# k-flouris/cmf

Measured on AMD Instinct MI355X. Metric: log-density evals/sec (JtJ-cholesky path), MNIST D=784 d=64 bs=512, higher is better.
Workload: dtype f32 (3x3 tangent convs as bf16x3 split MFMA, fp32 accumulate); 1 GPU; C3: MNIST-shaped (1,28,28) uint8-range + U[0,1) noise, non-square flow d=64, cholesky J^T J log-det + g_ij off-diagonal L1 + reconstruction, eval/no_grad; per_gpu_batch=512, global_batch=512, D=784, latent_dimension=64, parallelism=dp1

## Files before the change

### cmf_amd/_lib.py

```python
import ctypes as C
import os
import threading

_HERE = os.path.dirname(os.path.abspath(__file__))
LIB_PATH = os.path.join(_HERE, "libcmf_amd.so")

F_NONE, F_RELU, F_TANH, F_RAW, F_SELF_RELU, F_RELU_BITS = 0, 1, 2, 3, 4, 5
O_NONE, O_TANH, O_STANH = 0, 1, 2

_fp = C.c_void_p
_ll = C.c_longlong
_i = C.c_int
_f = C.c_float
_d = C.c_double


class ConvTangentArgs(C.Structure):
    _fields_ = [("x", _fp), ("x_np", _ll), ("x_ci", _ll), ("x_px", _ll),
                ("f", _fp), ("f_np", _ll), ("f_ci", _ll), ("f_px", _ll), ("fmode", _i),
                ("w", _fp),
                ("y", _fp), ("y_np", _ll), ("y_co", _ll), ("y_px", _ll),
                ("r", _fp), ("r_np", _ll), ("r_co", _ll), ("r_px", _ll),
                ("np", _i), ("cin", _i), ("cout", _i), ("H", _i), ("W", _i), ("nc", _i), ("taps", _i),
                ("bias", _fp), ("f_group", _i), ("x_sl", _ll), ("y_sl", _ll), ("r_sl", _ll),
                ("fo", _fp), ("fo_np", _ll), ("fo_co", _ll), ("fo_px", _ll), ("fomode", _i),
                ("mask_out", _fp), ("mask_np", _ll), ("amax_in", _fp), ("amax_out", _fp), ("live", _i),
                ("ymask", _fp), ("ymask_np", _ll),
                ("head_w", _fp), ("head_cout", _i), ("head_a", _fp), ("head_a_np", _ll), ("head_a_c", _ll), ("head_a_px", _ll),
                ("head_y", _fp), ("head_y_np", _ll), ("head_y_co", _ll), ("head_y_px", _ll)]


class ConvPrimalArgs(C.Structure):
    _fields_ = [("x", _fp), ("x_b", _ll), ("x_c", _ll), ("x_px", _ll),
                ("f", _fp), ("f_c", _ll), ("f_px", _ll), ("imode", _i),
                ("w", _fp), ("bias", _fp), ("sw", _fp), ("sb", _fp),
                ("y", _fp), ("y_b", _ll), ("y_c", _ll), ("y_px", _ll),
                ("g", _fp),
                ("r", _fp), ("r_b", _ll), ("r_c", _ll), ("r_px", _ll),
                ("omode", _i),
                ("B", _i), ("cin", _i), ("cout", _i), ("H", _i), ("W", _i), ("taps", _i)]


class ProbeApplyArgs(C.Structure):
    _fields_ = [("r", _fp), ("r_np", _ll), ("r_px", _ll),
# ... 12 lines not shown
    _fields_ = [("z", _fp), ("z_b", _ll), ("t", _fp), ("t_f", _ll), ("w", _fp),
                ("zi", _fp), ("si", _fp), ("ti", _fp), ("n_mod", _i),
                ("B", _i), ("cin", _i), ("chan_off", _i), ("chan_step", _i), ("n_layers", _i),
                ("width", _i * (MLP_MAX_LAYERS + 1)), ("w_off", _ll * MLP_MAX_LAYERS), ("decode", _i), ("lj", _fp), ("ncols", _i)]


SIGNATURES = {
    "cmf_version": (C.c_char_p, []),
    "cmf_pack_weight": (_i, [_fp, _fp, _i, _i, _i, _i, C.POINTER(_ll), _fp]),
    "cmf_pack_weights_batched": (_i, [_fp, _i, _fp]),
    "cmf_conv_tangent": (_i, [C.POINTER(ConvTangentArgs), _fp]),
    "cmf_pack_weight_bf16x3": (_i, [_fp, _fp, _i, _i, C.POINTER(_ll), _fp]),
    "cmf_pack_weight_bf16x3_t": (_i, [_fp, _fp, _i, _i, _i, C.POINTER(_ll), _fp]),
    "cmf_conv_tangent_bf16x3": (_i, [C.POINTER(ConvTangentArgs), _fp]),
    "cmf_probe_apply": (_i, [C.POINTER(ProbeApplyArgs), _fp]),
    "cmf_pack_weight_f16x3": (_i, [_fp, _fp, _i, _i, _i, C.POINTER(_ll), _fp]),
    "cmf_conv_tangent_f16x3": (_i, [C.POINTER(ConvTangentArgs), _fp]),
    "cmf_conv_tangent_f16x3_item": (_i, [C.POINTER(ConvTangentArgs), _i, _fp]),
    "cmf_absmax": (_i, [_fp, _ll, _fp, _fp]),
    "cmf_conv_tangent_wgrad_ws": (_ll, [C.POINTER(ConvTangentArgs)]),
    "cmf_conv_tangent_wgrad": (_i, [C.POINTER(ConvTangentArgs), _fp, _fp, _fp, _ll, _fp]),
    "cmf_conv_tangent_wgrad_bf16x3": (_i, [C.POINTER(ConvTangentArgs), _fp, _fp, _fp, _ll, _fp]),
    "cmf_conv_tangent_wgrad_bf16x3_batched": (_i, [C.POINTER(ConvTangentArgs), _i, C.POINTER(_fp), C.POINTER(_fp), C.POINTER(_fp), _fp, _ll, _fp]),
    "cmf_primal_regroup": (_i, [_fp, _fp, _i, _ll, _i, _fp]),
    "cmf_conv_primal": (_i, [C.POINTER(ConvPrimalArgs), _fp]),
    "cmf_acl_primal": (_i, [_fp, _ll, _fp, _ll, _fp, _fp, _fp, _i, _i, _i, _fp, _fp]),
    "cmf_acl_tangent": (_i, [_fp, _ll, _ll, _fp, _ll, _ll, _i, _fp, _ll, _fp, _ll, _fp, _fp, _fp, _fp, _i, _i, _fp]),
    "cmf_acl_cotangent": (_i, [_fp, _ll, _ll, _fp, _ll, _ll, _i, _fp, _ll, _fp, _ll, _fp, _fp, _fp, _fp, _i, _i, _fp]),
    "cmf_acl_primal_backward": (_i, [_fp, _ll, _fp, _ll, _fp, _ll, _fp, _fp, _fp, _fp, _i, _i, _i, _fp, _fp]),
    "cmf_acl_cross_terms": (_i, [_fp, _ll, _ll, _fp, _ll, _ll, _fp, _ll, _ll, _i, _fp, _ll, _fp, _ll, _fp, _fp, _fp, _fp, _i, _i,
# ... 138 lines not shown
```

### cmf_amd/csrc/conv_tangent_bf16x3.hip

```cpp
#include <cstdlib>
#include <type_traits>
#include "common.h"

#ifdef CMF_DBG_STAMP
__device__ unsigned long long cmf_dbg_stamps[3][64][4];
extern "C" int cmf_debug_read_stamps(void* out) {
  return (int)hipMemcpyFromSymbol(out, HIP_SYMBOL(cmf_dbg_stamps), sizeof(cmf_dbg_stamps));
}
#define STAMP(role, g, k)                                                                        \
  do {                                                                                            \
    if (blockIdx.x == 0 && (g) < 64 && lane == 0 && wave == ((role) == 1 ? 4 : 0)) {                   \
      unsigned long long t_;                                                                      \
      asm volatile("s_memtime %0\n\ts_waitcnt lgkmcnt(0)" : "=s"(t_)::"memory");                  \
      cmf_dbg_stamps[role][g][k] = t_;                                                            \
    }                                                                                             \
  } while (0)
__device__ unsigned long long cmf_dbg_wg_span[1024][2];
extern "C" int cmf_debug_read_wg_span(void* out) {
  return (int)hipMemcpyFromSymbol(out, HIP_SYMBOL(cmf_dbg_wg_span), sizeof(cmf_dbg_wg_span));
}
#define SPAN(k)                                                                                   \
  do {                                                                                            \
    if (lane == 0 && wave == 0 && blockIdx.x < 1024) {                                            \
      unsigned long long t_;                                                                      \
// ... 67 lines not shown

__device__ __forceinline__ int xslot(int col, int pix) { return (((col & 3) << 2) + (col >> 2) + ((pix & 1) << 2)) & 15; }

template <int COT, int PXW, int MODE, bool F16 = false, bool FRES = false, bool CKB = false>
__global__ __launch_bounds__(512, 2) void conv_tangent_bf16x3_kernel(cmf_conv_tangent_args a, int tiles_x, int ntiles,
                                                                       int nslices, int ncog, int total) {
  static_assert(!CKB || (!F16 && !FRES && (MODE == 1 || MODE == 3)), "checkerboard output: the forward tangent conv with a relu' factor");
  static_assert(!F16 || ((MODE == 2 || MODE == 4) && (COT == 4 || COT == 2)), "the fp16 variant is the primal pass: SELF mode (forward) or 4 (backward)");
  constexpr bool BWD = F16 && MODE == 4;
  static_assert(!BWD || FRES, "the backward form uses the epilogue with tile loads");
  constexpr bool HALF = F16 && COT == 2;
  constexpr int COG = HALF ? 32 : 64;
  static_assert(!FRES || F16, "residual-in-the-epilogue is the fp16 variant's");
  constexpr bool YMASK = !F16 && (MODE == 6 || MODE == 7);
  static_assert(!YMASK || (COT == 4 && !CKB), "the store filter: whole 64-channel groups, every pixel");
  constexpr bool SELF = MODE == 2, RELU = MODE == 1 || MODE == 6, BITS = MODE == 3 || MODE == 7;
  constexpr bool PLAIN = !F16 && (MODE == 4 || MODE == 5);
  constexpr bool INPLACE = MODE == 5;
  constexpr bool NOF = SELF || PLAIN || BWD;
  constexpr int NF = NOF ? 0 : BITS ? 1 : 8;
  using C = BCfg<COT, PXW>;
  constexpr int CW = COT / 2, PW = CKB ? C::PW / 2 : C::PW;
  auto tp = [](int p) constexpr { return CKB ? 2 * p : p; };
  auto trow = [&](int p) constexpr { return tp(p) / C::TW; };
  static_assert(COT % 2 == 0, "the co-split wave layout needs an even number of output-channel tiles");
  extern __shared__ __attribute__((aligned(16))) unsigned char smem[];

  const int tid = threadIdx.x, lane = tid & 63;
  const int wave = __builtin_amdgcn_readfirstlane(tid >> 6);
  const bool loader = wave >= 4;
  SPAN(0);
// ... 424 lines not shown
    coff_ring[1] = ck_o[1] ? r1 + 256 : r0;
    coff_stage[0] = ck_o[0] ? s1 + 256 : s0;
    coff_stage[1] = ck_o[1] ? s1 + 256 : s0;
  }
  const int aoff = (lane << 4) + ((cohalf * CW * 64) << 4);

#ifdef CMF_DBG_BD
  constexpr int BD = CMF_DBG_BD;
#else
  constexpr int BD = PW > 14 ? 3 : 4;
#endif

  typedef unsigned bu32x4 __attribute__((vector_size(16)));
  constexpr int RS_FLAGS = 0x00020000;
  const int yvoff = 4 * ((cohalf * CW * 16 + cl) * y_co + kq * 4);
  const int rvoff = 4 * ((cohalf * CW * 16 + cl) * r_co + kq * 4);
  struct Item {
    int ypix, rpix;
    int pix0, np, cog;
  };
  auto item_geom = [&](int item, int& np, int& slice, int& cog, Item& it) {
    int tile;
    decode(item, tile, slice, cog, np);
    const int pix0 = (C::TH * (tile / tiles_x) + wrow) * a.W + C::TW * (tile % tiles_x);
    it.ypix = CKB ? 4 * ((C::TH * (tile / tiles_x) + wrow) * (a.W / 2) + C::TW / 2 * (tile % tiles_x)) * y_px
                  : 4 * pix0 * y_px;
    it.rpix = 4 * pix0 * r_px;
    it.pix0 = pix0, it.np = np, it.cog = cog;
  };
  typedef int i32x4 __attribute__((ext_vector_type(4)));
  auto y_rsrc = [&](int np, int slice, int cog) {
    const unsigned long long u = reinterpret_cast<unsigned long long>(a.y + (long long)np * a.y_np + (long long)slice * (a.y_sl ? a.y_sl : 16) + (long long)cog * COG * y_co);
    const unsigned lo = __builtin_amdgcn_readfirstlane((int)(unsigned)u);
    const unsigned hi = __builtin_amdgcn_readfirstlane((int)(unsigned)(u >> 32));
    return __builtin_amdgcn_make_buffer_rsrc(reinterpret_cast<float*>(((unsigned long long)hi << 32) | lo), 0, 0x7fffff00, RS_FLAGS);
  };
  constexpr int Y_DROP = 0x7ffffff0;
  [[maybe_unused]] auto m_rsrc = [&](int np, int slice, int cog) {
    const unsigned long long u = reinterpret_cast<unsigned long long>(a.mask_out ? a.mask_out : (void*)a.y) +
                                 (unsigned long long)((long long)np * a.nc + slice * 16) * a.mask_np + (unsigned)(cog * (COG / 8) + cohalf * (COG / 16));
    const unsigned lo = __builtin_amdgcn_readfirstlane((int)(unsigned)u);
    const unsigned hi = __builtin_amdgcn_readfirstlane((int)(unsigned)(u >> 32));
    return __builtin_amdgcn_make_buffer_rsrc(reinterpret_cast<float*>(((unsigned long long)hi << 32) | lo), 0,
                                             a.mask_out ? 0x7fffff00 : 0, RS_FLAGS);
  };
  const int mvoff = lane < 16 ? lane * (int)a.mask_np : Y_DROP;
  float ymax = 0.f;
  auto r_rsrc = [&](int np, int slice, int cog, bool on) {
    const float* base = a.r ? a.r + (long long)np * a.r_np + (long long)slice * (a.r_sl ? a.r_sl : 16) + (long long)cog * COG * r_co : a.y;
    const unsigned long long u = reinterpret_cast<unsigned long long>(base);
    i32x4 d;
    d[0] = __builtin_amdgcn_readfirstlane((int)(unsigned)u);
    d[1] = __builtin_amdgcn_readfirstlane((int)((unsigned)(u >> 32) & 0xffffu));
    d[2] = __builtin_amdgcn_readfirstlane((a.r && on) ? -1 : 0);
    d[3] = RS_FLAGS;
    return d;
  };
  f32x4 acc[PW][CW];
  Item cur, nxt;
  int np_, slice_, cog_;
  item_geom(0, np_, slice_, cog_, cur);
  nxt.ypix = cur.ypix, nxt.rpix = cur.rpix, nxt.pix0 = cur.pix0, nxt.np = cur.np, nxt.cog = cur.cog;
  float bias[CW];
  [[maybe_unused]] float bias_h1 = 0.f;
  {
    const unsigned long long u = reinterpret_cast<unsigned long long>(a.bias ? a.bias : a.y);
    i32x4 d;
    d[0] = __builtin_amdgcn_readfirstlane((int)(unsigned)u);
    d[1] = __builtin_amdgcn_readfirstlane((int)((unsigned)(u >> 32) & 0xffffu));
    d[2] = __builtin_amdgcn_readfirstlane(a.bias ? -1 : 0);
    d[3] = RS_FLAGS;
    const int bvo = 4 * (cohalf * CW * 16 + cl);
#pragma unroll
    for (int c = 0; c < CW; ++c) {
      const int so = 4 * c * 16;
      asm volatile("s_nop 4\n\tbuffer_load_dword %0, %1, %2, %3 offen" : "=v"(bias[c]) : "v"(bvo), "s"(d), "s"(so) : "memory");
    }
    if constexpr (HALF) {
      const int so = 4 * 32;
      asm volatile("s_nop 4\n\tbuffer_load_dword %0, %1, %2, %3 offen" : "=v"(bias_h1) : "v"(bvo), "s"(d), "s"(so) : "memory");
    }
  }
  auto cur_yrs = y_rsrc(np_, slice_, cog_);
  auto cur_mrs = cur_yrs;
  if constexpr (F16) cur_mrs = m_rsrc(np_, slice_, cog_);
  i32x4 nxt_rrs = r_rsrc(np_, slice_, cog_, n_items > 0);
  auto init_pixel = [&](const Item& it, const i32x4& rrs_in, int p) __attribute__((always_inline)) {
    i32x4 rrs;
#pragma unroll
    for (int i = 0; i < 4; ++i) rrs[i] = __builtin_amdgcn_readfirstlane(rrs_in[i]);
#pragma unroll
    for (int c = 0; c < CW; ++c) {
      const int so = it.rpix + 4 * ((trow(p) * a.W + tp(p) % C::TW + (CKB ? ck_o[trow(p) & 1] : 0)) * r_px + c * 16 * r_co);
      asm volatile("s_nop 4\n\tbuffer_load_dwordx4 %0, %1, %2, %3 offen" : "=v"(acc[p][c]) : "v"(rvoff), "s"(rrs), "s"(so) : "memory");
    }
  };
  unsigned omask[PW];
  const bool use_omask = PLAIN && a.fomode == CMF_F_RELU_BITS;
  constexpr bool inplace = INPLACE;
  auto load_omask = [&](const Item& it) __attribute__((always_inline)) {
    if constexpr (PLAIN || YMASK) {
      const unsigned long long base = (YMASK ? reinterpret_cast<unsigned long long>(a.ymask) + (unsigned long long)it.np * a.ymask_np
                                             : reinterpret_cast<unsigned long long>(a.fo) + (unsigned long long)it.np * a.fo_np) +
                                      (unsigned)(it.cog * 8 + cohalf * 4);
      const unsigned lo = __builtin_amdgcn_readfirstlane((int)(unsigned)base);
// ... 76 lines not shown
            "s_pack_hh_b32_b16 %3, %1, vcc_lo\n\t"
            "v_writelane_b32 %0, %3, %7\n\t"
            "s_pack_ll_b32_b16 %3, %2, vcc_hi\n\t"
            "v_writelane_b32 %0, %3, %8\n\t"
            "s_pack_hh_b32_b16 %3, %2, vcc_hi\n\t"
            "v_writelane_b32 %0, %3, %9"
            : "+v"(mbits), "=&s"(alo), "=&s"(ahi), "=&s"(d)
            : "v"(vst[0][r]), "v"(vst[1][r]), "n"(r), "n"(4 + r), "n"(8 + r), "n"(12 + r)
            : "vcc");
      }
      __builtin_amdgcn_raw_buffer_store_b32(mbits, cur_mrs, mvoff, (it.pix0 + (p / C::TW) * a.W + p % C::TW) * (a.cout / 8), 0);
    }
  };
  auto wait_res = [&](int p, bool also_last) __attribute__((always_inline)) {
    static_assert(CW == 2 || CW == 1, "operand list below");
    constexpr int NT = 2 * CW + (F16 ? 1 : 0);
    const int n0 = NT * (PW - 1 - p) + (also_last ? NT * p : 0);
    const int n = n0 > 63 ? 63 : n0;
    if constexpr (CW == 2) asm volatile("s_waitcnt vmcnt(%2)" : "+v"(acc[p][0]), "+v"(acc[p][1]) : "n"(n));
    else asm volatile("s_waitcnt vmcnt(%1)" : "+v"(acc[p][0]) : "n"(n));
  };

  int g = 0;
  auto chunk = [&](int stage, int ring_slot, auto FIRST, auto LAST, auto QUAD) __attribute__((always_inline)) {
#ifdef CMF_DBG_NOMFMA
    if (LAST) {
#pragma unroll
      for (int p = 0; p < PW; ++p) {
        store_pixel(cur, p, f32x4{}, f32x4{});
        init_pixel(nxt, nxt_rrs, p);
      }
    }
    return;
#endif
    constexpr int KS = QUAD ? 3 : 2, NSTEP = KS * PW;
    if (LAST) load_omask(cur);
    const unsigned char* Xh = smem + stage * C::BUF_BYTES;
    const unsigned char* Xl = Xh + C::XS_BYTES;
    const unsigned char* Wh = Xh + 2 * C::XS_BYTES;
    const unsigned char* Wl = Wh + C::WS_BYTES;
    bf16x8 ah[KS][CW], al[KS][CW], bh[BD], bl[BD];
    const unsigned char* ch_[2];
    const unsigned char* cl_[2];
    if (QUAD) {
#pragma unroll
      for (int par = 0; par < 2; ++par) {
        ch_[par] = smem + (kq < 3 ? coff_ring[par] : stage * C::BUF_BYTES + coff_stage[par]);
        cl_[par] = smem + (kq < 3 ? coff_ring[par] + C::RING_HALF : stage * C::BUF_BYTES + C::XS_BYTES + coff_stage[par]);
      }
    }
    auto load_b = [&](int t) {
      const int s = t % KS, p = t / KS;
#ifdef CMF_DBG_NOLDS
      asm volatile("" : "=v"(bh[t % BD]), "=v"(bl[t % BD]));
      return;
#endif
// ... 37 lines not shown
      if (t + BD - 1 < NSTEP) load_b(t + BD - 1);
#ifndef CMF_DBG_NORING
      if (!QUAD && t == 2) {
        unsigned char* dst = smem + 2 * C::BUF_BYTES + ring_slot * C::RING_SLOT + (cohalf ? C::RING_HALF : 0) + wrow * C::TW * 256;
#pragma unroll
        for (int k = 0; k < 4; ++k) {
          const int u = lane + 64 * k;
          if (u < C::PW * 16) *reinterpret_cast<u32x4*>(dst + u * 16) = cp[k];
        }
      }
#endif
      if (FIRST && s == 0 && FRES) {
#pragma unroll
        for (int c = 0; c < CW; ++c) acc[p][c] = f32x4{0.f, 0.f, 0.f, 0.f};
      }
      if (FIRST && s == 0 && !FRES) {
#ifndef CMF_DBG_SPREAD
        wait_res(p, false);
#endif
        if constexpr (F16) {
#pragma unroll
          for (int c = 0; c < CW; ++c) acc[p][c] *= rscale;
        }
      }
#pragma unroll
      for (int c = 0; c < CW; ++c) {
        if constexpr (F16) {
#define CMF_H8(v) __builtin_bit_cast(f16x8, v)
          acc[p][c] = __builtin_amdgcn_mfma_f32_16x16x32_f16(CMF_H8(bh[t % BD]), CMF_H8(al[s][c]), acc[p][c], 0, 0, 0);
          acc[p][c] = __builtin_amdgcn_mfma_f32_16x16x32_f16(CMF_H8(bl[t % BD]), CMF_H8(ah[s][c]), acc[p][c], 0, 0, 0);
          acc[p][c] = __builtin_amdgcn_mfma_f32_16x16x32_f16(CMF_H8(bh[t % BD]), CMF_H8(ah[s][c]), acc[p][c], 0, 0, 0);
// ... 167 lines not shown
#pragma unroll
  for (int o = 32; o > 0; o >>= 1) m = fmaxf(m, __shfl_xor(m, o, 64));
  if ((threadIdx.x & 63) == 0) red[threadIdx.x >> 6] = m;
  __syncthreads();
  if (threadIdx.x == 0) {
    for (int i = 1; i < 16; ++i) m = fmaxf(m, red[i]);
    const int ex = (int)((__builtin_bit_cast(unsigned, m) >> 23) & 0xffu);
    int k = (ex == 0 || ex == 255) ? 0 : 12 - (ex - 126);
    k = k < -60 ? -60 : k > 60 ? 60 : k;
    trailer[0] = pow2i(k);
    trailer[1] = pow2i(-k);
    trailer[2] = trailer[3] = 0.f;
  }
}

template <int COT, int PXW, int MODE, bool F16 = false, bool FRES = false, bool CKB = false>
int launch(const cmf_conv_tangent_args& a, hipStream_t s) {
  using C = BCfg<COT, PXW>;
  const int tiles_x = cmf_ceil_div(a.W, C::TW), tiles = tiles_x * cmf_ceil_div(a.H, C::TH);
  const int nslices = a.nc / 16, ncog = (F16 && COT == 2) ? a.cout / 32 : cmf_ceil_div(a.cout, 64);
  const long long total = (long long)tiles * nslices * ncog * a.np;
  if (total > 0x7fffffffLL) return CMF_ERANGE;
  auto k = conv_tangent_bf16x3_kernel<COT, PXW, MODE, F16, FRES, CKB>;
  constexpr int lds = C::LDS_BYTES;
  if (hipError_t e = cmf_set_dynamic_lds((const void*)k, lds); e != hipSuccess) return (int)e;
  const int n_cu = cmf_device_cus();
  int grid = (int)(total < n_cu ? total : n_cu);
#ifdef CMF_DBG_STAMP
  if (const char* e = getenv("CMF_DBG_GRID")) grid = atoi(e) < grid ? atoi(e) : grid;
#endif
  hipLaunchKernelGGL(k, dim3(grid), dim3(512), lds, s, a, tiles_x, tiles, nslices, ncog, (int)total);
  CMF_LAUNCH_CHECK();
  return 0;
}

template <int PXW>
int launch_cot(const cmf_conv_tangent_args& a, hipStream_t s) {
  if (a.ymask) return a.fmode == CMF_F_RELU ? launch<4, PXW, 6>(a, s) : launch<4, PXW, 7>(a, s);
  if (a.fmode == CMF_F_SELF_RELU) return (a.cout > 32) ? launch<4, PXW, 2>(a, s) : launch<2, PXW, 2>(a, s);
// ... 10 lines not shown

}

extern "C" int cmf_pack_weight_bf16x3_t(const float* w, void* out, int cout, int cin, int transpose, long long* out_bytes, void* stream);
extern "C" int cmf_pack_weight_bf16x3(const float* w, void* out, int cout, int cin, long long* out_bytes, void* stream) {
  return cmf_pack_weight_bf16x3_t(w, out, cout, cin, 0, out_bytes, stream);
}
extern "C" int cmf_pack_weight_bf16x3_t(const float* w, void* out, int cout, int cin, int transpose, long long* out_bytes, void* stream) {
  if (cout <= 0 || cin <= 0 || cin % 8) return CMF_EINVAL;
  const long long total = (long long)((cout + 63) / 64) * (cin / 8) * 2 * 3 * 4 * 4 * 16 * 8;
  if (out_bytes) *out_bytes = total * 2;
  if (!out) return 0;
  if (!w) return CMF_EINVAL;
  hipLaunchKernelGGL(pack_weight_bf16x3_kernel, dim3((unsigned)((total + 255) / 256)), dim3(256), 0, (hipStream_t)stream,
                     w, (unsigned short*)out, cout, cin, total, transpose ? 1 : 0, 0);
  CMF_LAUNCH_CHECK();
  return 0;
}

extern "C" int cmf_pack_weight_f16x3(const float* w, void* out, int cout, int cin, int transpose, long long* out_bytes, void* stream) {
  if (cout <= 0 || cin <= 0 || cin % 8) return CMF_EINVAL;
  const long long total = (long long)((cout + 63) / 64) * (cin / 8) * 2 * 3 * 4 * 4 * 16 * 8;
  if (out_bytes) *out_bytes = total * 2 + 16;
  if (!out) return 0;
  if (!w || (uintptr_t)out % 16) return CMF_EINVAL;
  hipLaunchKernelGGL(pack_f16_scale_kernel, dim3(1), dim3(1024), 0, (hipStream_t)stream, w, (long long)cout * cin * 9,
                     reinterpret_cast<float*>((unsigned short*)out + total));
  CMF_LAUNCH_CHECK();
  hipLaunchKernelGGL(pack_weight_bf16x3_kernel, dim3((unsigned)((total + 255) / 256)), dim3(256), 0, (hipStream_t)stream,
                     w, (unsigned short*)out, cout, cin, total, transpose ? 1 : 0, 1);
// ... 22 lines not shown
    if (a.ymask_np % 4 || (uintptr_t)a.ymask % 4 || a.ymask_np < (long long)a.H * a.W * (a.cout / 8)) return CMF_EINVAL;
  }
  if ((a.x_np | a.x_ci | a.x_px | a.x_sl | a.y_sl | a.r_sl) % 4 || ((uintptr_t)a.x % 16) || ((uintptr_t)a.w % 16)) return CMF_EINVAL;
  if ((a.y_np | a.y_co | a.y_px) % 4 || ((uintptr_t)a.y % 16)) return CMF_EINVAL;
  if (a.r && ((a.r_np | a.r_co | a.r_px) % 4 || ((uintptr_t)a.r % 16))) return CMF_EINVAL;
  const long long HW = (long long)a.H * a.W;
  if (!fits_int((a.cin + 8) * a.x_ci + HW * a.x_px + a.nc) || !fits_int((a.cin + 8) * a.f_ci + HW * a.f_px) ||
      !fits_int((a.cout + 64) * a.y_co + HW * a.y_px + a.nc + 64) ||
      (a.r && !fits_int((a.cout + 64) * a.r_co + HW * a.r_px + a.nc)) ||
      HW > (1 << 24))
    return CMF_ERANGE;
  hipStream_t s = (hipStream_t)stream;
  const bool t14 = a.W % 14 == 0 && a.H % 2 == 0, t8 = a.W % 8 == 0 && a.H % 4 == 0;
  if (!(t14 || t8) || !(a.cout % 64 == 0 || a.cout == 32)) return CMF_EINVAL;
  if (a.bias && a.cout > 64) return CMF_EINVAL;
  if (a.live) {
    if (a.live < 0 || a.live > 2 || (a.fmode != CMF_F_RELU && a.fmode != CMF_F_RELU_BITS) || a.fo || a.bias || a.cout % 64 || a.W % 2)
      return CMF_EINVAL;
    if (a.fmode == CMF_F_RELU) return t14 ? launch<4, 7, 1, false, false, true>(a, s) : launch<4, 4, 1, false, false, true>(a, s);
    return t14 ? launch<4, 7, 3, false, false, true>(a, s) : launch<4, 4, 3, false, false, true>(a, s);
  }
  if (a.fmode == CMF_F_NONE && !a.fo) {
    cmf_conv_tangent_args b = a;
    b.fo = a.x;
    b.fo_np = 0;
    b.fomode = CMF_F_NONE;
    return t14 ? launch_cot<7>(b, s) : launch_cot<4>(b, s);
  }
  return t14 ? launch_cot<7>(a, s) : launch_cot<4>(a, s);
}
// ... 43 lines not shown
```

### cmf_amd/engine.py

```python
import ctypes as C
import threading

import numpy as np
import torch
import torch.nn as nn

from . import _lib
from ._lib import (F_NONE, F_RELU, F_TANH, F_RAW, F_SELF_RELU, F_RELU_BITS, O_NONE, O_TANH, O_STANH, ConvPrimalArgs,
                   ConvTangentArgs)


def _stream():
    return C.c_void_p(torch.cuda.current_stream().cuda_stream)


def _p(t):
    return None if t is None else C.c_void_p(t.data_ptr())


def require_gpu(t, what="input"):
    if not t.is_cuda:
        raise RuntimeError(f"cmf_amd: {what} is on {t.device}; the log-density path runs only through the HIP "
                           "kernels on an AMD GPU (there is no CPU fallback)")
    if t.dtype != torch.float32:
# ... 285 lines not shown
    a = ConvPrimalArgs()
    a.x = C.c_void_p(x_ptr_t.data_ptr() + 4 * int(x_off)); a.x_b, a.x_c, a.x_px = int(x_b), int(x_c), int(x_px)
    a.f = _p(mask); a.f_c, a.f_px = int(f_c), int(f_px); a.imode = imode
    a.w = _p(PACKS.get(weight, taps)); a.bias = _p(bias); a.sw = _p(sw); a.sb = _p(sb)
    a.y = _p(y); a.y_b, a.y_c, a.y_px = int(y_b), int(y_c), int(y_px)
    a.g = _p(g)
    a.r = _p(res); a.r_b, a.r_c, a.r_px = int(y_b), int(y_c), int(y_px)
    a.omode = omode
    a.B, a.cin, a.cout, a.H, a.W, a.taps = int(B), int(cin), int(cout), int(H), int(W), int(taps)
    _lib.check(lib.cmf_conv_primal(C.byref(a), _stream()), "cmf_conv_primal")


def conv_tangent(x_t, x_off, x_np, x_ci, x_px, weight, taps, y_t, y_np, y_co, y_px, np_, cin, cout, H, W, nc,
                 fmode=F_NONE, f=None, f_np=0, f_ci=0, f_px=0, res_t=None, transpose=False, bias=None, f_group=1,
                 x_sl=16, y_sl=16, precision=None, y_off=0, res_off=0, fo=None, fo_np=0, fo_co=0, fo_px=0, fomode=F_NONE,
                 mask_out=None, mask_np=0, amax_in=None, amax_out=None, item_channels=0, live=0, res_np=None, ymask=None, head=None):
    lib = _lib.load()
    a = ConvTangentArgs()
    if head is not None:
        assert (precision or cfg().tangent) == "bf16x3" and not transpose and bias is None and fo is None and ymask is None \
            and mask_out is None, "the folded head replaces the split-precision forward conv + 1x1 conv only"
        return _conv_tangent_head(lib, a, x_t, x_off, x_np, x_ci, x_px, weight, taps, y_t, y_np, y_co, y_px, np_, cin, cout, H, W, nc,
                                  fmode, f, f_np, res_t, res_off, res_np, x_sl, y_off, live, head)
    a.x = C.c_void_p(x_t.data_ptr() + 4 * int(x_off)); a.x_np, a.x_ci, a.x_px = int(x_np), int(x_ci), int(x_px)
    a.f = _p(f); a.f_np, a.f_ci, a.f_px = int(f_np), int(f_ci), int(f_px); a.fmode = fmode
    obits = isinstance(fo, BitMask)
    inplace = res_t is not None and res_t.data_ptr() == y_t.data_ptr() and int(res_off) == int(y_off)
    precision = precision or cfg().tangent
    split = (precision == "bf16x3" and _shape_ok_bf16x3(taps, cin, W, transpose, H, cout)
             and not (bias is not None and cout > 64)
             and ((fmode != F_NONE and fo is None) or
# ... 7 lines not shown
        fo, fo_np, fo_co, fo_px, fomode = fo.data, fo.np_bytes, 0, 0, F_RELU_BITS
    a.w = _p(PACKS.get(weight, taps, transpose, bf16x3="f16x3" if f16 else split))
    a.y = C.c_void_p(y_t.data_ptr() + 4 * int(y_off)); a.y_np, a.y_co, a.y_px = int(y_np), int(y_co), int(y_px)
    a.r = None if res_t is None else C.c_void_p(res_t.data_ptr() + 4 * int(res_off))
    a.r_np, a.r_co, a.r_px = int(y_np if res_np is None else res_np), int(y_co), int(y_px)
    a.fo = _p(fo); a.fo_np, a.fo_co, a.fo_px, a.fomode = int(fo_np), int(fo_co), int(fo_px), int(fomode)
    a.mask_out = _p(mask_out); a.mask_np = int(mask_np)
    assert not (fmode == F_RELU_BITS and not split), "bit-mask factors are read by the split-precision kernel only"
    assert not (mask_out is not None and split), "sign bits are written by the fp32 and the fp16-split kernels only"
    a.amax_in, a.amax_out = (_p(amax_in), _p(amax_out)) if f16 else (None, None)
    a.live = int(live)
    assert not live or split, "checkerboard output is the split-precision kernel's"
    assert ymask is None or split, "the store filter is the split-precision kernel's"
    if ymask is not None:
        a.ymask, a.ymask_np = _p(ymask.data), int(ymask.np_bytes)
    a.np, a.cin, a.cout, a.H, a.W, a.nc, a.taps = int(np_), int(cin), int(cout), int(H), int(W), int(nc), int(taps)
    a.bias = _p(bias); a.f_group = int(f_group)
    a.x_sl, a.y_sl, a.r_sl = int(x_sl), int(y_sl), int(y_sl)
    fn, what = ((lib.cmf_conv_tangent_f16x3, "cmf_conv_tangent_f16x3") if f16 else
                (lib.cmf_conv_tangent_bf16x3, "cmf_conv_tangent_bf16x3") if split else (lib.cmf_conv_tangent, "cmf_conv_tangent"))
    launch = lambda: _lib.check(fn(C.byref(a), _stream()), what)
    if f16 and item_channels:
        launch = lambda: _lib.check(lib.cmf_conv_tangent_f16x3_item(C.byref(a), int(item_channels), _stream()), "cmf_conv_tangent_f16x3_item")
    if fmode == F_SELF_RELU and not f16 and _lib.tracing():
        run = launch

        def launch():
            with _lib.role("primal"):
                run()
    TIMER = _timer()
    if TIMER is None:
        return launch()
    px_in = float(H) * W * nc * np_
    px = px_in * (0.5 if live else 1.0)
    TIMER.wrap(f"conv_tangent_t{taps}_ci{cin}_co{cout}" + ("_primal" if fmode == F_SELF_RELU else "_primal_bwd" if pbwd else "_live" if live else ""),
               2.0 * cin * cout * taps * px,
               4.0 * (px_in * cin + px * (cout + (cout if res_t is not None else 0))), launch)


def _conv_tangent_head(lib, a, x_t, x_off, x_np, x_ci, x_px, weight, taps, y_t, y_np, y_co, y_px, np_, cin, cout, H, W, nc, fmode, f,
                       f_np, res_t, res_off, res_np, x_sl, y_off, live, head):
    wf, act = head["weight"], head["act"]
    hc = int(wf.shape[0])
    w2, wf = weight.detach(), wf.detach().reshape(hc, -1)
    assert w2.is_contiguous() and wf.is_contiguous() and act.is_contiguous() and w2.dtype == wf.dtype == act.dtype == torch.float32
    a.x = C.c_void_p(x_t.data_ptr() + 4 * int(x_off)); a.x_np, a.x_ci, a.x_px, a.x_sl = int(x_np), int(x_ci), int(x_px), int(x_sl)
    a.f = _p(f); a.f_np = int(f_np); a.fmode = int(fmode)
    a.w = _p(w2)
    a.r = None if res_t is None else C.c_void_p(res_t.data_ptr() + 4 * int(res_off))
    a.r_np, a.r_co, a.r_px, a.r_sl = int(x_np if res_np is None else res_np), int(x_ci), int(x_px), int(x_sl)
    a.np, a.cin, a.cout, a.H, a.W, a.nc, a.taps, a.live = int(np_), int(cin), int(cout), int(H), int(W), int(nc), int(taps), int(live)
    a.head_w, a.head_cout = _p(wf), hc
# ... 962 lines not shown


CHECKERBOARD_TAIL = True

SKIP_DEAD_ROWS = True

FOLD_HEAD = True


PROBE_FRONT = True

PROBE_FRONT_SHAPES = {(28, 28, 1)}

PROBE_CLASSES = 13


def probe_plan(mask):
    mask = np.asarray(mask)
    if mask.ndim != 3:
        return None
    cin, H, W = mask.shape
    if not 1 <= cin <= 2:
        return None
    r, col = np.meshgrid(np.arange(H), np.arange(W), indexing="ij")
    cls = (np.mod(r - 5 * col, 2 * PROBE_CLASSES) >> 1)[None] + PROBE_CLASSES * np.arange(cin)[:, None, None]
    cls = np.where(mask != 0, cls, -1).astype(np.int8)
    for r0 in range(H):
        for c0 in range(W):
            win = cls[:, max(r0 - 2, 0):r0 + 3, max(c0 - 2, 0):c0 + 3].reshape(-1)
            win = win[win >= 0]
# ... 12 lines not shown
    a.r = _p(R); a.r_np, a.r_px = int(r_np), int(r_px)
    a.t = C.c_void_p(T.data_ptr() + 4 * int(t_off)); a.t_np, a.t_c, a.t_px = int(t_np), int(t_c), int(t_px)
    a.cls = _p(cls)
    a.y = _p(y); a.y_np, a.y_px = int(y_np), int(y_px)
    if ymask is not None:
        a.ymask, a.ymask_np = _p(ymask.data), int(ymask.np_bytes)
    a.np, a.cin, a.H, a.W, a.nc, a.ns = int(np_), int(cin), int(H), int(W), int(nc), int(ns)
    launch = lambda: _lib.check(_lib.load().cmf_probe_apply(C.byref(a), _stream()), "cmf_probe_apply")
    TIMER = _timer()
    if TIMER is None:
        return launch()
    px = float(H) * W * np_
    TIMER.wrap(f"probe_apply_ci{cin}", 2.0 * PROBE_CLASSES * cin * 64 * nc * px, 4.0 * px * 64 * (nc + 16 * ns), launch)


def _probe_hidden(conv0, view, plan, H, W, hid, dev):
    HW, ncp = H * W, 16 * plan["ns"]

    def build():
        out = torch.empty(HW * hid * ncp, dtype=torch.float32, device=dev)
        conv_tangent(plan["probes"], 0, view.cin * HW * ncp, HW * ncp, ncp, conv0.weight, 9, out, hid * HW * ncp, 16, hid * ncp,
                     1, view.cin, hid, H, W, ncp, fmode=F_RAW, f=view.mask, f_np=0, f_ci=HW, f_px=1, y_sl=hid * 16)
        return out

    return DERIVED.get((id(conv0.weight), "probe-front", H, W, view.cin, str(dev)), [conv0.weight], build)


def probe_front(conv0, conv1, T, view, plan, factor, ymask, scratch, u, H, W):
    B, nc, HW, hid, dev = T.B, T.nc, H * W, conv1.out_channels, T.data.device
    assert hid == 64 and T.layout == "panel"
# ... 3 lines not shown
    probe_apply(scratch, hid * HW * ncp, hid * ncp, T.data, view.chan_off * HW * nc, T.t_b, view.chan_step * HW * nc, nc,
                plan["cls"], u, hid * HW * nc, hid * nc, B, view.cin, H, W, nc, plan["ns"], ymask=ymask)


def net_tangent(net, T, view, acts, transpose_packs=False, save=None):
    geo, B, nc, dev = view.geom, T.B, T.nc, T.data.device
    if save is not None:
        save.append(_view_rows(T, view))
    if net.kind == "resnet":
        conv0, blocks, convf = _resnet_parts(net)
        hid, cout, H, W, HW = conv0.out_channels, convf.out_channels, geo.H, geo.W, geo.HW
        new = lambda c: Tangent(B, c * HW, nc, "panel", dev)
        pn = lambda c: (c * HW * nc, HW * nc, nc)
        hd = (hid * HW * nc, 16, hid * nc)
        hsl = hid * 16
        h = new(hid)
        conv_tangent(T.data, view.chan_off * HW * nc, T.t_b, view.chan_step * HW * nc, nc, conv0.weight, 9, h.data, *hd,
                     B, view.cin, hid, H, W, nc, fmode=F_RAW if view.mask is not None else F_NONE, f=view.mask, f_np=0,
                     f_ci=HW, f_px=1, y_sl=hsl)
        fg = getattr(acts, "f_group", 1)
        fs = dict(f_np=hid * HW * fg, f_ci=HW * fg, f_px=fg, f_group=fg)
        fk = lambda t: dict(fmode=F_RELU_BITS, f=t.data, f_np=t.np_bytes) if isinstance(t, BitMask) else dict(fmode=F_RELU, f=t, **fs)
        u, h2 = new(hid), new(hid)
        compact = (CHECKERBOARD_TAIL and view.live is not None and save is None and fg == 1 and len(blocks) > 0 and hid % 64 == 0
                   and W % 2 == 0 and _use_bf16x3(9, hid, W, False, H, hid))
        filt = SKIP_DEAD_ROWS and save is None and hid % 64 == 0 and _use_bf16x3(9, hid, W, False, H, hid)
        fold = (FOLD_HEAD and view.live is not None and save is None and fg == 1 and len(blocks) > 0 and hid == 64 and cout <= 8 and nc % 16 == 0
                and isinstance(acts[2 * len(blocks) - 1], BitMask) and _use_bf16x3(9, hid, W, False, H, hid))
        plan = getattr(view, "probe", None)
        probe = (PROBE_FRONT and plan is not None and save is None and fg == 1 and len(blocks) > 0 and hid == 64 and view.mask is not None
                 and T.layout == "panel" and nc % 16 == 0 and nc > 16 * plan["ns"] and (H, W, view.cin) in PROBE_FRONT_SHAPES
                 and cfg().tangent == "bf16x3" and _use_bf16x3(9, hid, W, False, H, hid))
        for k, blk in enumerate(blocks):
            a_in, c1 = acts[2 * k], acts[2 * k + 1]
            ym = c1 if filt and isinstance(c1, BitMask) else None
            if probe and k == 0:
                probe_front(conv0, blk.conv1, T, view, plan, fk(a_in), ym, h2.data, u.data, H, W)
            else:
                conv_tangent(h.data, 0, *hd, blk.conv1.weight, 9, u.data, *hd, B, hid, hid, H, W, nc, x_sl=hsl, y_sl=hsl, **fk(a_in),
                             ymask=ym)
            if fold and k + 1 == len(blocks):
                HWo = HW // 2 if compact else HW
                yt = Tangent(B, cout * HWo, nc, "panel", dev)
                conv_tangent(u.data, 0, *hd, blk.conv2.weight, 9, yt.data, cout * HWo * nc, HWo * nc, nc, B, hid, hid, H, W, nc,
                             res_t=h.data, res_np=hd[0], x_sl=hsl, live=view.live["parity"] if compact else 0,
                             head=dict(weight=convf.weight, act=acts[-1]), **fk(c1))
                if compact:
                    yt.compact = True
                return yt
            if compact and k + 1 == len(blocks):
                HWc = HW // 2
                hc = Tangent(B, hid * HWc, nc, "panel", dev)
                conv_tangent(u.data, 0, *hd, blk.conv2.weight, 9, hc.data, hid * HWc * nc, 16, hid * nc, B, hid, hid, H, W, nc,
                             res_t=h.data, res_np=hd[0], x_sl=hsl, y_sl=hsl, live=view.live["parity"], **fk(c1))
                a_last = gather_primal(acts[-1], view.live["act_idx"], hid * HWc)
# ... 266 lines not shown
```

### include/cmf_amd.h

```cpp
#ifndef CMF_AMD_H
#define CMF_AMD_H

#ifdef __cplusplus
extern "C" {
#endif

#define CMF_EINVAL (-1)
#define CMF_ERANGE (-2)

#define CMF_F_NONE 0
#define CMF_F_RELU 1
#define CMF_F_TANH 2
#define CMF_F_RAW  3
#define CMF_F_SELF_RELU 4
#define CMF_F_RELU_BITS 5

#define CMF_O_NONE  0
#define CMF_O_TANH  1
#define CMF_O_STANH 2

const char* cmf_version(void);

int cmf_pack_weight(const float* w, float* out, int cout, int cin, int taps, int transpose,
                    long long* out_floats, void* stream);
// ... 11 lines not shown
  const float* w;
  float* y;       long long y_np, y_co, y_px;
  const float* r; long long r_np, r_co, r_px;
  int np, cin, cout, H, W, nc, taps;
  const float* bias;
  int f_group;
  long long x_sl, y_sl, r_sl;
  const float* fo; long long fo_np, fo_co, fo_px; int fomode;
  void* mask_out; long long mask_np;
  const float* amax_in; float* amax_out;
  int live;
  const void* ymask; long long ymask_np;
  const float* head_w; int head_cout;
  const float* head_a; long long head_a_np, head_a_c, head_a_px;
  float* head_y; long long head_y_np, head_y_co, head_y_px;
} cmf_conv_tangent_args;
int cmf_conv_tangent(const cmf_conv_tangent_args* a, void* stream);

int cmf_pack_weight_bf16x3(const float* w, void* out, int cout, int cin, long long* out_bytes, void* stream);
int cmf_pack_weight_bf16x3_t(const float* w, void* out, int cout, int cin, int transpose, long long* out_bytes, void* stream);
int cmf_conv_tangent_bf16x3(const cmf_conv_tangent_args* a, void* stream);

typedef struct {
  const float* r; long long r_np, r_px;
  const float* t; long long t_np, t_c, t_px;
  const signed char* cls;
  float* y;       long long y_np, y_px;
  const void* ymask; long long ymask_np;
  int np, cin, H, W, nc, ns;
} cmf_probe_apply_args;
int cmf_probe_apply(const cmf_probe_apply_args* a, void* stream);

int cmf_pack_weight_f16x3(const float* w, void* out, int cout, int cin, int transpose, long long* out_bytes, void* stream);
int cmf_conv_tangent_f16x3(const cmf_conv_tangent_args* a, void* stream);
int cmf_conv_tangent_f16x3_item(const cmf_conv_tangent_args* a, int item_channels, void* stream);
int cmf_absmax(const float* x, long long n, float* out, void* stream);
// ... 150 lines not shown
```

Baseline: 1496 evals/s.

## Fold first 1-channel tangent conv into block residual via seeded MFMA epilogue

Measured after the change: 1511 evals/s, median of 6. 1.01x the previous value.

```diff
diff --git a/cmf_amd/_lib.py b/cmf_amd/_lib.py
--- a/cmf_amd/_lib.py
+++ b/cmf_amd/_lib.py
@@ -27,7 +27,8 @@
                 ("mask_out", _fp), ("mask_np", _ll), ("amax_in", _fp), ("amax_out", _fp), ("live", _i),
                 ("ymask", _fp), ("ymask_np", _ll),
                 ("head_w", _fp), ("head_cout", _i), ("head_a", _fp), ("head_a_np", _ll), ("head_a_c", _ll), ("head_a_px", _ll),
-                ("head_y", _fp), ("head_y_np", _ll), ("head_y_co", _ll), ("head_y_px", _ll)]
+                ("head_y", _fp), ("head_y_np", _ll), ("head_y_co", _ll), ("head_y_px", _ll),
+                ("seed", _fp), ("seed_np", _ll), ("seed_col", _ll), ("seed_w", _fp)]
 
 
 class ConvPrimalArgs(C.Structure):
@@ -70,6 +71,8 @@
     "cmf_pack_weight_bf16x3_t": (_i, [_fp, _fp, _i, _i, _i, C.POINTER(_ll), _fp]),
     "cmf_conv_tangent_bf16x3": (_i, [C.POINTER(ConvTangentArgs), _fp]),
     "cmf_probe_apply": (_i, [C.POINTER(ProbeApplyArgs), _fp]),
+    "cmf_pack_seed_weight": (_i, [_fp, _fp, _fp]),
+    "cmf_seed_panel": (_i, [_fp, _ll, _ll, _fp, _fp, _ll, _ll, _i, _i, _i, _i, _fp]),
     "cmf_pack_weight_f16x3": (_i, [_fp, _fp, _i, _i, _i, C.POINTER(_ll), _fp]),
     "cmf_conv_tangent_f16x3": (_i, [C.POINTER(ConvTangentArgs), _fp]),
     "cmf_conv_tangent_f16x3_item": (_i, [C.POINTER(ConvTangentArgs), _i, _fp]),
diff --git a/cmf_amd/csrc/conv_tangent_bf16x3.hip b/cmf_amd/csrc/conv_tangent_bf16x3.hip
--- a/cmf_amd/csrc/conv_tangent_bf16x3.hip
+++ b/cmf_amd/csrc/conv_tangent_bf16x3.hip
@@ -105,7 +105,9 @@
   static_assert(!FRES || F16, "residual-in-the-epilogue is the fp16 variant's");
   constexpr bool YMASK = !F16 && (MODE == 6 || MODE == 7);
   static_assert(!YMASK || (COT == 4 && !CKB), "the store filter: whole 64-channel groups, every pixel");
-  constexpr bool SELF = MODE == 2, RELU = MODE == 1 || MODE == 6, BITS = MODE == 3 || MODE == 7;
+  constexpr bool SELF = MODE == 2, RELU = MODE == 1 || MODE == 6, BITS = MODE == 3 || MODE == 7 || MODE == 8;
+  constexpr bool RSEED = !F16 && MODE == 8;
+  static_assert(!RSEED || (COT == 4 && PXW == 7 && !CKB), "the seeded residual: 64-channel groups on 2 x 14 tiles, every pixel");
   constexpr bool PLAIN = !F16 && (MODE == 4 || MODE == 5);
   constexpr bool INPLACE = MODE == 5;
   constexpr bool NOF = SELF || PLAIN || BWD;
@@ -560,7 +562,7 @@
   typedef unsigned bu32x4 __attribute__((vector_size(16)));
   constexpr int RS_FLAGS = 0x00020000;
   const int yvoff = 4 * ((cohalf * CW * 16 + cl) * y_co + kq * 4);
-  const int rvoff = 4 * ((cohalf * CW * 16 + cl) * r_co + kq * 4);
+  const int rvoff = RSEED ? (kq < 3 ? 4 * (cl * (int)a.seed_col + kq * (a.W + 2)) : 0x7ffffff0) : 4 * ((cohalf * CW * 16 + cl) * r_co + kq * 4);
   struct Item {
     int ypix, rpix;
     int pix0, np, cog;
@@ -571,7 +573,8 @@
     const int pix0 = (C::TH * (tile / tiles_x) + wrow) * a.W + C::TW * (tile % tiles_x);
     it.ypix = CKB ? 4 * ((C::TH * (tile / tiles_x) + wrow) * (a.W / 2) + C::TW / 2 * (tile % tiles_x)) * y_px
                   : 4 * pix0 * y_px;
-    it.rpix = 4 * pix0 * r_px;
+    it.rpix = RSEED ? 4 * ((C::TH * (tile / tiles_x) + wrow) * (a.W + 2) + C::TW * (tile % tiles_x))
+                    : 4 * pix0 * r_px;
     it.pix0 = pix0, it.np = np, it.cog = cog;
   };
   typedef int i32x4 __attribute__((ext_vector_type(4)));
@@ -593,12 +596,13 @@
   const int mvoff = lane < 16 ? lane * (int)a.mask_np : Y_DROP;
   float ymax = 0.f;
   auto r_rsrc = [&](int np, int slice, int cog, bool on) {
-    const float* base = a.r ? a.r + (long long)np * a.r_np + (long long)slice * (a.r_sl ? a.r_sl : 16) + (long long)cog * COG * r_co : a.y;
+    const float* base = RSEED ? a.seed + (long long)np * a.seed_np + (long long)slice * 16 * a.seed_col
+                        : a.r ? a.r + (long long)np * a.r_np + (long long)slice * (a.r_sl ? a.r_sl : 16) + (long long)cog * COG * r_co : a.y;
     const unsigned long long u = reinterpret_cast<unsigned long long>(base);
     i32x4 d;
     d[0] = __builtin_amdgcn_readfirstlane((int)(unsigned)u);
     d[1] = __builtin_amdgcn_readfirstlane((int)((unsigned)(u >> 32) & 0xffffu));
-    d[2] = __builtin_amdgcn_readfirstlane((a.r && on) ? -1 : 0);
+    d[2] = __builtin_amdgcn_readfirstlane(RSEED ? (on ? 0x7fffff00 : 0) : (a.r && on) ? -1 : 0);
     d[3] = RS_FLAGS;
     return d;
   };
@@ -627,6 +631,18 @@
       asm volatile("s_nop 4\n\tbuffer_load_dword %0, %1, %2, %3 offen" : "=v"(bias_h1) : "v"(bvo), "s"(d), "s"(so) : "memory");
     }
   }
+  if constexpr (RSEED) {
+    const unsigned long long u = reinterpret_cast<unsigned long long>(a.seed_w);
+    i32x4 d;
+    d[0] = __builtin_amdgcn_readfirstlane((int)(unsigned)u);
+    d[1] = __builtin_amdgcn_readfirstlane((int)((unsigned)(u >> 32) & 0xffffu));
+    d[2] = 4096;
+    d[3] = RS_FLAGS;
+    u32x4 t;
+    const int vo = tid << 4, so = 0;
+    asm volatile("s_nop 4\n\tbuffer_load_dwordx4 %0, %1, %2, %3 offen\n\ts_waitcnt vmcnt(0)" : "=&v"(t) : "v"(vo), "s"(d), "s"(so) : "memory");
+    *reinterpret_cast<u32x4*>(smem + C::LDS_BYTES + (tid << 4)) = t;
+  }
   auto cur_yrs = y_rsrc(np_, slice_, cog_);
   auto cur_mrs = cur_yrs;
   if constexpr (F16) cur_mrs = m_rsrc(np_, slice_, cog_);
@@ -635,6 +651,11 @@
     i32x4 rrs;
 #pragma unroll
     for (int i = 0; i < 4; ++i) rrs[i] = __builtin_amdgcn_readfirstlane(rrs_in[i]);
+    if constexpr (RSEED) {
+      const int so = __builtin_amdgcn_readfirstlane(it.rpix + 4 * (trow(p) * (a.W + 2) + tp(p) % C::TW));
+      asm volatile("s_nop 4\n\tbuffer_load_dwordx4 %0, %1, %2, %3 offen" : "=v"(acc[p][0]) : "v"(rvoff), "s"(rrs), "s"(so) : "memory");
+      return;
+    }
 #pragma unroll
     for (int c = 0; c < CW; ++c) {
       const int so = it.rpix + 4 * ((trow(p) * a.W + tp(p) % C::TW + (CKB ? ck_o[trow(p) & 1] : 0)) * r_px + c * 16 * r_co);
@@ -741,10 +762,11 @@
   };
   auto wait_res = [&](int p, bool also_last) __attribute__((always_inline)) {
     static_assert(CW == 2 || CW == 1, "operand list below");
-    constexpr int NT = 2 * CW + (F16 ? 1 : 0);
+    constexpr int NT = RSEED ? CW + 1 : 2 * CW + (F16 ? 1 : 0);
     const int n0 = NT * (PW - 1 - p) + (also_last ? NT * p : 0);
     const int n = n0 > 63 ? 63 : n0;
-    if constexpr (CW == 2) asm volatile("s_waitcnt vmcnt(%2)" : "+v"(acc[p][0]), "+v"(acc[p][1]) : "n"(n));
+    if constexpr (RSEED) asm volatile("s_waitcnt vmcnt(%1)" : "+v"(acc[p][0]) : "n"(n));
+    else if constexpr (CW == 2) asm volatile("s_waitcnt vmcnt(%2)" : "+v"(acc[p][0]), "+v"(acc[p][1]) : "n"(n));
     else asm volatile("s_waitcnt vmcnt(%1)" : "+v"(acc[p][0]) : "n"(n));
   };
 
@@ -767,6 +789,13 @@
     const unsigned char* Wh = Xh + 2 * C::XS_BYTES;
     const unsigned char* Wl = Wh + C::WS_BYTES;
     bf16x8 ah[KS][CW], al[KS][CW], bh[BD], bl[BD];
+    [[maybe_unused]] f32x4 sw[CW];
+    if constexpr (RSEED) {
+      if (FIRST) {
+#pragma unroll
+        for (int c = 0; c < CW; ++c) sw[c] = *reinterpret_cast<const f32x4*>(smem + C::LDS_BYTES + (((cohalf * CW + c) * 64 + lane) << 4));
+      }
+    }
     const unsigned char* ch_[2];
     const unsigned char* cl_[2];
     if (QUAD) {
@@ -834,7 +863,19 @@
 #pragma unroll
         for (int c = 0; c < CW; ++c) acc[p][c] = f32x4{0.f, 0.f, 0.f, 0.f};
       }
-      if (FIRST && s == 0 && !FRES) {
+      if constexpr (RSEED) {
+        if (FIRST && s == 0) {
+          wait_res(p, false);
+          const float s0 = acc[p][0][0], s1 = acc[p][0][1], s2 = acc[p][0][2];
+#pragma unroll
+          for (int c = 0; c < CW; ++c) {
+            acc[p][c] = __builtin_amdgcn_mfma_f32_16x16x4f32(s0, sw[c][0], f32x4{0.f, 0.f, 0.f, 0.f}, 0, 0, 0);
+            acc[p][c] = __builtin_amdgcn_mfma_f32_16x16x4f32(s1, sw[c][1], acc[p][c], 0, 0, 0);
+            acc[p][c] = __builtin_amdgcn_mfma_f32_16x16x4f32(s2, sw[c][2], acc[p][c], 0, 0, 0);
+          }
+        }
+      }
+      if (FIRST && s == 0 && !FRES && !RSEED) {
 #ifndef CMF_DBG_SPREAD
         wait_res(p, false);
 #endif
@@ -1032,6 +1073,44 @@
   }
 }
 
+__global__ void pack_seed_weight_kernel(const float* __restrict__ w, float* __restrict__ out) {
+  const int i = blockIdx.x * 256 + threadIdx.x;
+  const int j = i & 3, lane = (i >> 2) & 63, cot = i >> 8;
+  const int kq = lane >> 4, co = cot * 16 + (lane & 15);
+  out[i] = (kq < 3 && j < 3) ? w[co * 9 + 3 * kq + j] : 0.f;
+}
+
+__global__ __launch_bounds__(256) void seed_panel_kernel(const float* __restrict__ v, long long v_np, long long v_px,
+                                                         const float* __restrict__ mask, float* __restrict__ out, long long o_np,
+                                                         int o_col, int H, int W, int nc) {
+  __shared__ float tile[64][17];
+  const int t = threadIdx.x, p0 = blockIdx.x * 64, c0 = blockIdx.y * 16;
+  const long long b = blockIdx.z;
+  {
+    const int col = t & 15;
+#pragma unroll
+    for (int i = 0; i < 4; ++i) {
+      const int pl = (t >> 4) + 16 * i, pp = p0 + pl;
+      const int r = pp / (W + 2) - 1, c = pp % (W + 2) - 1;
+      float x = 0.f;
+      if (r >= 0 && r < H && c >= 0 && c < W) {
+        const float m = mask ? mask[r * W + c] : 1.f;
+        if (m != 0.f) x = m * v[b * v_np + (long long)(r * W + c) * v_px + c0 + col];
+      }
+      tile[pl][col] = x;
+    }
+  }
+  __syncthreads();
+  const int pl = t & 63, pp = p0 + pl;
+  if (pp < o_col) {
+#pragma unroll
+    for (int j = 0; j < 4; ++j) {
+      const int col = (t >> 6) + 4 * j;
+      out[b * o_np + (long long)(c0 + col) * o_col + pp] = tile[pl][col];
+    }
+  }
+}
+
 template <int COT, int PXW, int MODE, bool F16 = false, bool FRES = false, bool CKB = false>
 int launch(const cmf_conv_tangent_args& a, hipStream_t s) {
   using C = BCfg<COT, PXW>;
@@ -1040,7 +1119,7 @@
   const long long total = (long long)tiles * nslices * ncog * a.np;
   if (total > 0x7fffffffLL) return CMF_ERANGE;
   auto k = conv_tangent_bf16x3_kernel<COT, PXW, MODE, F16, FRES, CKB>;
-  constexpr int lds = C::LDS_BYTES;
+  constexpr int lds = C::LDS_BYTES + (MODE == 8 ? 4096 : 0);
   if (hipError_t e = cmf_set_dynamic_lds((const void*)k, lds); e != hipSuccess) return (int)e;
   const int n_cu = cmf_device_cus();
   int grid = (int)(total < n_cu ? total : n_cu);
@@ -1081,6 +1160,23 @@
   if (!w) return CMF_EINVAL;
   hipLaunchKernelGGL(pack_weight_bf16x3_kernel, dim3((unsigned)((total + 255) / 256)), dim3(256), 0, (hipStream_t)stream,
                      w, (unsigned short*)out, cout, cin, total, transpose ? 1 : 0, 0);
+  CMF_LAUNCH_CHECK();
+  return 0;
+}
+
+extern "C" int cmf_pack_seed_weight(const float* w, void* out, void* stream) {
+  if (!w || !out || (uintptr_t)out % 16) return CMF_EINVAL;
+  hipLaunchKernelGGL(pack_seed_weight_kernel, dim3(4), dim3(256), 0, (hipStream_t)stream, w, (float*)out);
+  CMF_LAUNCH_CHECK();
+  return 0;
+}
+
+extern "C" int cmf_seed_panel(const float* v, long long v_np, long long v_px, const float* mask, float* out, long long out_np,
+                              long long out_col, int np, int H, int W, int nc, void* stream) {
+  if (!v || !out || np <= 0 || H <= 0 || W <= 0 || nc <= 0 || nc % 16 || v_px < nc) return CMF_EINVAL;
+  if (out_col < (long long)(H + 2) * (W + 2) + 1 || out_np < out_col * nc || out_col > (1 << 24) || np > 65535) return CMF_EINVAL;
+  hipLaunchKernelGGL(seed_panel_kernel, dim3((unsigned)((out_col + 63) / 64), nc / 16, np), dim3(256), 0, (hipStream_t)stream, v, v_np,
+                     v_px, mask, out, out_np, (int)out_col, H, W, nc);
   CMF_LAUNCH_CHECK();
   return 0;
 }
@@ -1133,6 +1229,13 @@
   const bool t14 = a.W % 14 == 0 && a.H % 2 == 0, t8 = a.W % 8 == 0 && a.H % 4 == 0;
   if (!(t14 || t8) || !(a.cout % 64 == 0 || a.cout == 32)) return CMF_EINVAL;
   if (a.bias && a.cout > 64) return CMF_EINVAL;
+  if (a.seed) {
+    if (!a.seed_w || a.r || a.fmode != CMF_F_RELU_BITS || a.cout != 64 || !t14 || a.live || a.ymask || a.fo || a.bias) return CMF_EINVAL;
+    if ((uintptr_t)a.seed % 4 || (uintptr_t)a.seed_w % 16) return CMF_EINVAL;
+    if (a.seed_col < (long long)(a.H + 2) * (a.W + 2) + 1 || a.seed_np < a.seed_col * a.nc) return CMF_EINVAL;
+    if (!fits_int(16 * a.seed_col)) return CMF_ERANGE;
+    return launch<4, 7, 8>(a, s);
+  }
   if (a.live) {
     if (a.live < 0 || a.live > 2 || (a.fmode != CMF_F_RELU && a.fmode != CMF_F_RELU_BITS) || a.fo || a.bias || a.cout % 64 || a.W % 2)
       return CMF_EINVAL;
diff --git a/cmf_amd/engine.py b/cmf_amd/engine.py
--- a/cmf_amd/engine.py
+++ b/cmf_amd/engine.py
@@ -323,7 +323,8 @@
 def conv_tangent(x_t, x_off, x_np, x_ci, x_px, weight, taps, y_t, y_np, y_co, y_px, np_, cin, cout, H, W, nc,
                  fmode=F_NONE, f=None, f_np=0, f_ci=0, f_px=0, res_t=None, transpose=False, bias=None, f_group=1,
                  x_sl=16, y_sl=16, precision=None, y_off=0, res_off=0, fo=None, fo_np=0, fo_co=0, fo_px=0, fomode=F_NONE,
-                 mask_out=None, mask_np=0, amax_in=None, amax_out=None, item_channels=0, live=0, res_np=None, ymask=None, head=None):
+                 mask_out=None, mask_np=0, amax_in=None, amax_out=None, item_channels=0, live=0, res_np=None, ymask=None, head=None,
+                 seed=None):
     lib = _lib.load()
     a = ConvTangentArgs()
     if head is not None:
@@ -361,6 +362,9 @@
     assert ymask is None or split, "the store filter is the split-precision kernel's"
     if ymask is not None:
         a.ymask, a.ymask_np = _p(ymask.data), int(ymask.np_bytes)
+    if seed is not None:
+        assert split and res_t is None and fmode == F_RELU_BITS, "the seeded residual is the split-precision kernel's, bit-mask factor"
+        a.seed, a.seed_np, a.seed_col, a.seed_w = _p(seed["panel"]), int(seed["np"]), int(seed["col"]), _p(seed["pack"])
     a.np, a.cin, a.cout, a.H, a.W, a.nc, a.taps = int(np_), int(cin), int(cout), int(H), int(W), int(nc), int(taps)
     a.bias = _p(bias); a.f_group = int(f_group)
     a.x_sl, a.y_sl, a.r_sl = int(x_sl), int(y_sl), int(y_sl)
@@ -381,8 +385,9 @@
     px_in = float(H) * W * nc * np_
     px = px_in * (0.5 if live else 1.0)
     TIMER.wrap(f"conv_tangent_t{taps}_ci{cin}_co{cout}" + ("_primal" if fmode == F_SELF_RELU else "_primal_bwd" if pbwd else "_live" if live else ""),
-               2.0 * cin * cout * taps * px,
-               4.0 * (px_in * cin + px * (cout + (cout if res_t is not None else 0))), launch)
+               2.0 * (cin + (1 if seed is not None else 0)) * cout * taps * px,
+               4.0 * (px_in * cin + px * (cout + (cout if res_t is not None else 0))
+                      + (float(seed["np"]) * np_ if seed is not None else 0.0)), launch)
 
 
 def _conv_tangent_head(lib, a, x_t, x_off, x_np, x_ci, x_px, weight, taps, y_t, y_np, y_co, y_px, np_, cin, cout, H, W, nc, fmode, f,
@@ -1375,6 +1380,8 @@
 
 PROBE_CLASSES = 13
 
+SEED_RESIDUAL = True
+
 
 def probe_plan(mask):
     mask = np.asarray(mask)
@@ -1417,6 +1424,52 @@
     TIMER.wrap(f"probe_apply_ci{cin}", 2.0 * PROBE_CLASSES * cin * 64 * nc * px, 4.0 * px * 64 * (nc + 16 * ns), launch)
 
 
+def seed_plane(H, W):
+    return ((H + 2) * (W + 2) + 1 + 3) // 4 * 4
+
+
+def seed_panel(T, view, H, W):
+    assert T.layout == "panel" and view.cin == 1
+    B, nc, HW, col = T.B, T.nc, H * W, seed_plane(H, W)
+    out = torch.empty(B * nc * col, dtype=torch.float32, device=T.data.device)
+    v = C.c_void_p(T.data.data_ptr() + 4 * int(view.chan_off * HW * nc))
+    launch = lambda: _lib.check(_lib.load().cmf_seed_panel(v, T.t_b, nc, _p(view.mask), _p(out), nc * col, col, B, H, W, nc, _stream()),
+                                "cmf_seed_panel")
+    TIMER = _timer()
+    if TIMER is None:
+        launch()
+    else:
+        TIMER.wrap("seed_panel", 0.0, 4.0 * B * nc * (col + HW), launch)
+    return dict(panel=out, np=nc * col, col=col)
+
+
+def seed_pack_host(w):
+    w = np.asarray(w, dtype=np.float32).reshape(64, 9)
+    out = np.zeros((4, 64, 4), dtype=np.float32)
+    for kq in range(3):
+        for j in range(3):
+            out[:, 16 * kq:16 * kq + 16, j] = w[:, 3 * kq + j].reshape(4, 16)
+    return out
+
+
+def seed_panel_index(H, W):
+    idx = np.full(seed_plane(H, W), -1, dtype=np.int64)
+    r, c = np.meshgrid(np.arange(H), np.arange(W), indexing="ij")
+    idx[((r + 1) * (W + 2) + c + 1).reshape(-1)] = (r * W + c).reshape(-1)
+    return idx
+
+
+def _seed_pack(conv0, dev):
+    def build():
+        w = conv0.weight.detach().contiguous()
+        assert tuple(w.shape) == (64, 1, 3, 3) and w.dtype == torch.float32
+        out = torch.empty(4096, dtype=torch.uint8, device=dev)
+        _lib.check(_lib.load().cmf_pack_seed_weight(_p(w), _p(out), _stream()), "cmf_pack_seed_weight")
+        return out
+
+    return DERIVED.get((id(conv0.weight), "seed-residual", str(dev)), [conv0.weight], build)
+
+
 def _probe_hidden(conv0, view, plan, H, W, hid, dev):
     HW, ncp = H * W, 16 * plan["ns"]
 
@@ -1450,10 +1503,6 @@
         pn = lambda c: (c * HW * nc, HW * nc, nc)
         hd = (hid * HW * nc, 16, hid * nc)
         hsl = hid * 16
-        h = new(hid)
-        conv_tangent(T.data, view.chan_off * HW * nc, T.t_b, view.chan_step * HW * nc, nc, conv0.weight, 9, h.data, *hd,
-                     B, view.cin, hid, H, W, nc, fmode=F_RAW if view.mask is not None else F_NONE, f=view.mask, f_np=0,
-                     f_ci=HW, f_px=1, y_sl=hsl)
         fg = getattr(acts, "f_group", 1)
         fs = dict(f_np=hid * HW * fg, f_ci=HW * fg, f_px=fg, f_group=fg)
         fk = lambda t: dict(fmode=F_RELU_BITS, f=t.data, f_np=t.np_bytes) if isinstance(t, BitMask) else dict(fmode=F_RELU, f=t, **fs)
@@ -1467,6 +1516,13 @@
         probe = (PROBE_FRONT and plan is not None and save is None and fg == 1 and len(blocks) > 0 and hid == 64 and view.mask is not None
                  and T.layout == "panel" and nc % 16 == 0 and nc > 16 * plan["ns"] and (H, W, view.cin) in PROBE_FRONT_SHAPES
                  and cfg().tangent == "bf16x3" and _use_bf16x3(9, hid, W, False, H, hid))
+        seeded = SEED_RESIDUAL and probe and view.cin == 1 and len(blocks) >= 2 and isinstance(acts[1], BitMask)
+        h = None
+        if not seeded:
+            h = new(hid)
+            conv_tangent(T.data, view.chan_off * HW * nc, T.t_b, view.chan_step * HW * nc, nc, conv0.weight, 9, h.data, *hd,
+                         B, view.cin, hid, H, W, nc, fmode=F_RAW if view.mask is not None else F_NONE, f=view.mask, f_np=0,
+                         f_ci=HW, f_px=1, y_sl=hsl)
         for k, blk in enumerate(blocks):
             a_in, c1 = acts[2 * k], acts[2 * k + 1]
             ym = c1 if filt and isinstance(c1, BitMask) else None
@@ -1475,6 +1531,12 @@
             else:
                 conv_tangent(h.data, 0, *hd, blk.conv1.weight, 9, u.data, *hd, B, hid, hid, H, W, nc, x_sl=hsl, y_sl=hsl, **fk(a_in),
                              ymask=ym)
+            if seeded and k == 0:
+                sd = seed_panel(T, view, H, W)
+                conv_tangent(u.data, 0, *hd, blk.conv2.weight, 9, h2.data, *hd, B, hid, hid, H, W, nc, x_sl=hsl, y_sl=hsl,
+                             seed=dict(sd, pack=_seed_pack(conv0, dev)), **fk(c1))
+                h, h2 = h2, new(hid)
+                continue
             if fold and k + 1 == len(blocks):
                 HWo = HW // 2 if compact else HW
                 yt = Tangent(B, cout * HWo, nc, "panel", dev)
diff --git a/include/cmf_amd.h b/include/cmf_amd.h
--- a/include/cmf_amd.h
+++ b/include/cmf_amd.h
@@ -49,12 +49,16 @@
   const float* head_w; int head_cout;
   const float* head_a; long long head_a_np, head_a_c, head_a_px;
   float* head_y; long long head_y_np, head_y_co, head_y_px;
+  const float* seed; long long seed_np, seed_col; const void* seed_w;
 } cmf_conv_tangent_args;
 int cmf_conv_tangent(const cmf_conv_tangent_args* a, void* stream);
 
 int cmf_pack_weight_bf16x3(const float* w, void* out, int cout, int cin, long long* out_bytes, void* stream);
 int cmf_pack_weight_bf16x3_t(const float* w, void* out, int cout, int cin, int transpose, long long* out_bytes, void* stream);
 int cmf_conv_tangent_bf16x3(const cmf_conv_tangent_args* a, void* stream);
+int cmf_pack_seed_weight(const float* w, void* out, void* stream);
+int cmf_seed_panel(const float* v, long long v_np, long long v_px, const float* mask, float* out, long long out_np, long long out_col,
+                   int np, int H, int W, int nc, void* stream);
 
 typedef struct {
   const float* r; long long r_np, r_px;
```
